# sagitrs/nvlevelz

Hardware: AMD Instinct MI355X
Metric: GiB/s device-resident batched CRC32C over 4 KiB blocks; % HBM-read roofline (higher is better)
Workload: dtype u32

## Files before the change

nvlevelz_amd/csrc/crc32c_dev_sched.h:

```cpp
#pragma once
#include "crc32c_dev.h"

namespace nvl {
namespace dev {

constexpr uint32_t kTail = 64;

template <int U, int NW = kWavesPerWG, int M = kAligned, class G = FixedGeom, bool kRaw = false, bool NIB = false>
__device__ __forceinline__ void run_pairs(const G& g, const KArgs& ka, uint8_t* lds) {
  NVL_STAMP0();
  const int lane = threadIdx.x & 63;
  const uint32_t wv = uniform_u32(threadIdx.x >> 6);
  const uint64_t B0 = g.n * blockIdx.x / gridDim.x;
  const uint64_t B1 = g.n * (blockIdx.x + 1) / gridDim.x;
  const uint32_t cnt = (uint32_t)(B1 - B0);
  const uint32_t nfull = cnt > kTail ? (cnt - kTail) / U : 0u;
  const uint32_t nunits = nfull + (cnt - nfull * U);

  auto unit_pos = [&](uint32_t u, int k, Pos& p) -> bool {
    const uint64_t i = u < nfull ? B0 + (uint64_t)u * U + (uint64_t)k : B0 + (uint64_t)nfull * U + (u - nfull);
    if (u >= nunits || (u >= nfull && k > 0)) return false;
    p.i = i;
    p.c = 0;
    p.bi = g.info(i);
    return true;
  };

  uint32_t u = wv;
  Pos gp[U];
  bool ok[U];
  Chunk cur[U];
  RegionFill rf;
  LdsFill<NW> lf;
  if constexpr (NIB) rf = fill_region_load(ka.tables);
  else lf = fill_lds_load<NW>(ka.tables);
#pragma unroll
  for (int k = 0; k < U; ++k) {
    ok[k] = unit_pos(u, k, gp[k]);
    if (ok[k]) load_chunk<M>(gp[k].bi, 0, lane, cur[k]);
  }
  if constexpr (NIB) fill_region_store(lds, rf, NW);
  else fill_lds_store<NW>(lds, lf, NW);
  __syncthreads();
  const LaneBase lb = make_lane_base(lane);
  NVL_STAMP1();

  while (u < nunits) {
    NVL_COUNT();
    const uint32_t un = pull_unit(lds, lane, NIB ? kRCtrOff : kCtrOff);
    Pos np[U];
    bool nok[U];
    Chunk nxt[U];
#pragma unroll
    for (int k = 0; k < U; ++k) {
      nok[k] = unit_pos(un, k, np[k]);
      if (nok[k]) load_chunk<M>(np[k].bi, 0, lane, nxt[k]);
    }
    if (ok[U - 1]) {
      BufInfo bis[U];
      uint32_t cs[U], raws[U];
#pragma unroll
      for (int k = 0; k < U; ++k) {
        bis[k] = gp[k].bi;
        cs[k] = 0;
      }
      group_raw<M, U, NIB>(lds, lb, bis, cs, lane, cur, raws);
      if (lane == 0) {
#pragma unroll
        for (int k = 0; k < U; ++k) {
          if constexpr (kRaw) ka.raws[gp[k].i] = raws[k];
          else ka.out[gp[k].i] = finish(~raws[k], ka.flags);
        }
      }
    } else {
#pragma unroll
      for (int k = 0; k < U; ++k) {
        if (ok[k]) {
          const uint32_t r = chunk_raw<M, NIB>(lds, lb, gp[k].bi, 0, lane, cur[k]);
          if (lane == 0) {
            if constexpr (kRaw) ka.raws[gp[k].i] = r;
            else ka.out[gp[k].i] = finish(~r, ka.flags);
          }
        }
      }
    }
    u = un;
#pragma unroll
    for (int k = 0; k < U; ++k) {
      gp[k] = np[k];
      ok[k] = nok[k];
      cur[k] = nxt[k];
    }
  }
  NVL_STAMP_END();
}

constexpr int kUnitStep = 1;
constexpr int kUnitStepAligned = 2;

template <int M, int NW, class G>
__device__ __forceinline__ void run_units(const G& g, const KArgs& ka, uint8_t* lds) {
  NVL_STAMP0();
  constexpr int kStep = M == kAligned ? kUnitStepAligned : kUnitStep;
  static_assert(M == kAligned || kStep == 1, "the kGeneral loop skips head chunks one step at a time");
  const int lane = threadIdx.x & 63;
  const uint32_t wv = uniform_u32(threadIdx.x >> 6);
  const uint64_t T = g.total();
  const uint32_t ub0 = blockIdx.x * kUnitsPerWG, ub1 = ub0 + kUnitsPerWG;
  constexpr bool kFastDiv = M != kAligned;
  auto lo_of = [&](uint32_t uu) -> uint64_t { return g.template unit_lo<kFastDiv>(T, uu); };
  auto skip = [&](const Pos& q) -> bool { return M == kGeneral && q.c == 0 && head_first(q.bi.len); };
  auto first_body = [&](const Pos& q) -> uint32_t { return (M == kGeneral && head_first(q.bi.len)) ? 1u : 0u; };
  auto hc_of = [&](const Pos& q) -> uint32_t {
    if (M != kGeneral || !ka.hc || q.c != 1u || !head_first(q.bi.len)) return 0u;
    return __builtin_nontemporal_load((const __attribute__((address_space(1))) uint32_t*)(ka.hc + q.i));
  };

  const LdsFill<NW> lf = fill_lds_load<NW>(ka.tables);
  uint32_t u = ub0 + wv;
  uint64_t t = lo_of(u), t1 = lo_of(u + 1);
  Pos p0{}, p1{};
  Chunk c0, c1;
  uint32_t hv0 = 0u;
  if (t < t1) {
    p0 = unit_start_pos<kFastDiv>(g, u, t);
    if (!skip(p0)) load_chunk<M>(p0.bi, p0.c, lane, c0);
    hv0 = hc_of(p0);
    if (kStep == 2 && t + 1 < t1) {
      p1 = next_pos(g, p0);
      load_chunk<M>(p1.bi, p1.c, lane, c1);
    }
  }
  fill_lds_store<NW>(lds, lf);
  __syncthreads();
  const LaneBase lb = make_lane_base(lane);
  NVL_STAMP1();

  uint32_t un = ub0 + pull_unit(lds, lane);
  uint64_t un_lo = un < ub1 ? lo_of(un) : 0, un_hi = un < ub1 ? lo_of(un + 1) : 0;
  UnitState st{0u, 0u, p0.c <= first_body(p0), Rec{kNoBuf, 0u, 0u}};
  Rec tail{kNoBuf, 0u, 0u};
  while (true) {
    const bool cur = t < t1;
    const bool two = kStep == 2 && t + 1 < t1;
    const uint64_t tn = cur ? t + (two ? 2u : 1u) : t;
    const bool unit_ends = tn == t1;
    Pos q0 = p0, q1 = p0;
    bool q0v = false, q1v = false;
    if (!unit_ends) {
      q0 = two ? next_pos(g, p1) : next_pos(g, p0);
      q0v = true;
      if (kStep == 2 && tn + 1 < t1) {
        q1 = next_pos(g, q0);
        q1v = true;
      }
    } else if (un_lo < un_hi) {
      q0 = unit_start_pos<kFastDiv>(g, un, un_lo);
      q0v = true;
      if (kStep == 2 && un_lo + 1 < un_hi) {
        q1 = next_pos(g, q0);
        q1v = true;
      }
    }
    const bool work = cur && !skip(p0);
    uint32_t w[2][16];
    uint32_t ov[2][4];
    if (work) {
      build_words<M>(p0.bi, p0.c, lane, c0, w[0], ov[0]);
      if (two) build_words<M>(p1.bi, p1.c, lane, c1, w[1], ov[1]);
    }
    Chunk n0, n1;
    uint32_t hvn = 0u;
    if (q0v && !skip(q0)) load_chunk<M>(q0.bi, q0.c, lane, n0);
    if (q0v) hvn = hc_of(q0);
    if (q1v) load_chunk<M>(q1.bi, q1.c, lane, n1);
    if (work) {
      NVL_COUNT();
      uint32_t r[2];
      if (two) {
        chains<2, false>(lds, lb, w, lane, r);
      } else {
        r[0] = chain_fold<M>(lds, lb, w[0], lane);
      }
      consume(st, p0, r[0], lds, lane, ka, hv0);
      if (two) consume(st, p1, r[1], lds, lane, ka);
    }
    if (unit_ends) {
      if (st.cnt) {
        const Pos& pl = two ? p1 : p0;
        const uint32_t norm = normalize(lds, ka.tables, st.acc, pl.bi.J - 1u - pl.c, lane);
        if (st.from_zero) tail = Rec{pl.i, norm, st.cnt};
        else st.head = Rec{pl.i, norm, st.cnt};
      }
      if (lane == 0) g.put_recs(ka, lds, u, st.head, tail);
      if (un >= ub1) break;
      u = un;
      t = un_lo;
      t1 = un_hi;
      un = ub0 + pull_unit(lds, lane);
      un_lo = un < ub1 ? lo_of(un) : 0;
      un_hi = un < ub1 ? lo_of(un + 1) : 0;
      st = UnitState{0u, 0u, q0.c <= first_body(q0), Rec{kNoBuf, 0u, 0u}};
      tail = Rec{kNoBuf, 0u, 0u};
    } else {
      t = tn;
    }
    p0 = q0;
    p1 = q1;
    c0 = n0;
    c1 = n1;
    hv0 = hvn;
  }
  NVL_STAMP_END();
}

template <int NW, class G>
__device__ __forceinline__ void run_general(const G& g, const KArgs& ka, uint8_t* lds) {
  run_units<kGeneral, NW>(g, ka, lds);
}

constexpr uint32_t kBufsMaxJ = 32;

struct CPos {
  uintptr_t ce;
  uint64_t i;
  uint32_t s;
  uint32_t f;
};
constexpr uint32_t kPosValid = 1u, kPosFirst = 2u, kPosLast = 4u, kPosHeadIn = 8u;

__device__ __forceinline__ void load_pos(const CPos& q, int lane, uintptr_t safe, const uint32_t* hc, Chunk& ch,
                                         uint32_t& hv) {
  const uint32_t r = (uint32_t)(q.ce & 3u);
  const uintptr_t A4 = q.ce - kChunk - r;
  const uint32_t lo = lane_load_off(lane);
#pragma unroll
  for (int j = 0; j < 4; ++j) {
    const u32x4 v = ld16(A4 + 1024u * (uint32_t)j + lo);
    ch.d[4 * j + 0] = v.x; ch.d[4 * j + 1] = v.y; ch.d[4 * j + 2] = v.z; ch.d[4 * j + 3] = v.w;
  }
  ch.e[3] = *(const __attribute__((address_space(1))) uint32_t*)(A4 + (r ? kChunk : kChunk - 4u));
  const uintptr_t ha = (q.f & kPosHeadIn) ? (uintptr_t)(hc + q.i) : safe;
  hv = __builtin_nontemporal_load((const __attribute__((address_space(1))) uint32_t*)ha);
}

__device__ __forceinline__ void build_pos(const CPos& q, int lane, const Chunk& ch, uint32_t (&w)[16]) {
#pragma unroll
  for (int k = 0; k < 16; ++k) w[k] = ch.d[k];
  row_transpose(w);
  const uint32_t r = (uint32_t)(q.ce & 3u);
  if (r != 0) {
    const uint32_t nx = next_lane(w[0], ch.e[3]);
#pragma unroll
    for (int k = 0; k < 15; ++k) w[k] = __builtin_amdgcn_alignbyte(w[k + 1], w[k], r);
    w[15] = __builtin_amdgcn_alignbyte(nx, w[15], r);
  }
  const uint32_t inj = q.f >> 8;
  if (inj < 4u && lane == 0) w[0] ^= q.s >> (8u * inj);
}

template <int NW, class G>
__device__ __forceinline__ void run_bufs(const G& g, const KArgs& ka, uint8_t* lds, uint64_t i0, uint64_t i1,
                                         const uint16_t* perm = nullptr) {
  NVL_STAMP0();
  const int lane = threadIdx.x & 63;
  const uint32_t wv = uniform_u32(threadIdx.x >> 6);
  const uint64_t nb = i1 > i0 ? i1 - i0 : 0;
constexpr int kBufsDiv = 4;
  const uint32_t GS = (uint32_t)max<uint64_t>(1, min<uint64_t>(kWave, nb / (kBufsDiv * NW)));
constexpr int kBufsTail = 0;
  const uint64_t kBT = kBufsTail;
  const uint64_t nbig = nb > kBT * 2 ? (nb - kBT) / GS : 0;
  const uint64_t ngroups = nbig + (nb - nbig * GS);
  const uintptr_t safe = (uintptr_t)ka.tables;

  uint64_t todo = 0;
  uintptr_t lp = 0;
  uint64_t lL = 0;
  uint32_t ls = 0, lr = 0;
  uint64_t ngb = 0;
  uint32_t ngn = 0;
  bool has_nxt = false, nxt_ready = false;
  uint64_t no = 0, nL = 0;
  uint32_t ni = 0, nr = 0;
  auto claim_group = [&](uint64_t k) {
    has_nxt = k < ngroups;
    nxt_ready = false;
    ngb = has_nxt ? i0 + (k < nbig ? k * GS : nbig * GS + (k - nbig)) : 0u;
    ngn = has_nxt ? (k < nbig ? GS : 1u) : 1u;
  };
  const uint32_t* const ibase = g.init ? g.init : reinterpret_cast<const uint32_t*>(safe);
  auto meta_load = [&]() {
    const uint64_t pos = ngb + (uint64_t)min<uint32_t>((uint32_t)lane, ngn - 1u);
    const uint64_t i = perm && pos >= i0 ? i0 + perm[pos - i0] : pos;
    nr = (uint32_t)(i - i0);
    no = g.offsets[i];
    nL = g.lengths[i];
    ni = ibase[g.init ? i : 0u];
  };
  auto adopt = [&]() {
    lp = (uintptr_t)g.base + no;
    lL = nL;
    ls = ~(g.init ? ni : g.init_all);
    lr = nr;
    todo = __ballot((uint32_t)lane < ngn && chunks_for(lL) > (head_first(lL) ? 1u : 0u));
    has_nxt = false;
  };
  uintptr_t cp = 0;
  uint64_t cL = 0, ci = 0;
  uint32_t cJ = 0, cx = 0, cc = 0, cfb = 0;
  bool cvalid = false;
  auto next_pos = [&](CPos& q) {
    q.ce = safe + kChunk;
    q.i = 0;
    q.s = 0;
    q.f = 0;
    if (cvalid && cc + 1u < cJ) {
      ++cc;
    } else {
      cvalid = false;
      while (todo == 0) {
        if (!has_nxt || !nxt_ready) return;
        adopt();
        claim_group(pull_unit(lds, lane));
      }
      const uint32_t j = (uint32_t)__builtin_ctzll(todo);
      todo &= todo - 1u;
      cp = (uintptr_t)lane_u64((uint64_t)lp, j);
      cL = lane_u64(lL, j);
      cx = lane_u32(ls, j);
      ci = i0 + lane_u32(lr, j);
      cJ = chunks_for(cL);
      cfb = head_first(cL) ? 1u : 0u;
      cc = cfb;
      cvalid = true;
    }
    q.ce = cp + cL - (uint64_t)kChunk * (cJ - 1u - cc);
    q.i = ci;
    q.s = cx;
    const uintptr_t cs = q.ce - kChunk;
    const uint32_t inj = cs < cp + 4u ? (uint32_t)(cs - cp) : 0xFFu;
    q.f = kPosValid | (cc == cfb ? kPosFirst : 0u) | (cc + 1u == cJ ? kPosLast : 0u) |
          (cc == cfb && cfb == 1u && ka.hc ? kPosHeadIn : 0u) | (inj << 8);
  };
  auto more = [&]() -> bool { return (cvalid && cc + 1u < cJ) || todo != 0 || has_nxt; };

  claim_group(wv);
  meta_load();
  if (has_nxt) adopt();
  claim_group(NW + wv);
  meta_load();
  CPos p0, p1;
  next_pos(p0);
  next_pos(p1);
  Chunk c0, c1;
  uint32_t hv0, hv1;
  const LdsFill<NW> lf = fill_lds_load<NW>(ka.tables);
  load_pos(p0, lane, safe, ka.hc, c0, hv0);
  load_pos(p1, lane, safe, ka.hc, c1, hv1);
  fill_lds_store<NW>(lds, lf, 2u * NW);
  __syncthreads();
  const LaneBase lb = make_lane_base(lane);
  NVL_STAMP1();
  uint32_t acc = 0u;
  auto accumulate = [&](const CPos& q, uint32_t raw, uint32_t hs) {
    const bool first = (q.f & kPosFirst) != 0u;
    acc = (first ? ((q.f & kPosHeadIn) ? hs : 0u) : shift4096(lds, acc, lane)) ^ raw;
    if ((q.f & kPosLast) && lane == 0) ka.out[q.i] = finish(~acc, ka.flags);
  };
  while (true) {
    nxt_ready = has_nxt;
    uint32_t w[2][16];
    const bool work = (p0.f & kPosValid) != 0u;
    if (work) {
      build_pos(p0, lane, c0, w[0]);
      build_pos(p1, lane, c1, w[1]);
    }
    const uint32_t hs0 = shift4096(lds, hv0, lane), hs1 = shift4096(lds, hv1, lane);
    CPos q0, q1;
    next_pos(q0);
    next_pos(q1);
    meta_load();
    load_pos(q0, lane, safe, ka.hc, c0, hv0);
    load_pos(q1, lane, safe, ka.hc, c1, hv1);
    if (work) {
      uint32_t raws[2];
      chains<2, false>(lds, lb, w, lane, raws);
      accumulate(p0, raws[0], hs0);
      if (p1.f & kPosValid) accumulate(p1, raws[1], hs1);
      NVL_COUNT();
    }
    if (!(q0.f & kPosValid) && !more()) break;
    p0 = q0;
    p1 = q1;
  }
  NVL_STAMP_END();
}


constexpr int kFastU = 2;

constexpr int kGenWaves = 16;
constexpr int kGenPairU = 2;
template <int M>
constexpr int waves_of() { return M == kGeneral ? kGenWaves : kWavesPerWG; }

constexpr uint32_t kMaxTiles = 1023;

}
}
```

nvlevelz_amd/csrc/crc32c_fixed.hip:

```cpp
#include "crc32c_launch.h"

namespace nvl {
namespace dev {

constexpr uint64_t kLongFixedMin = 1ull << 18;
__global__ __launch_bounds__(kThreads, 1) void crc32c_fixed_long_kernel(FixedGeom g, KArgs ka) {
  __shared__ __attribute__((aligned(16))) uint8_t lds[kLdsBytes > kRLdsBytes ? kLdsBytes : kRLdsBytes];
  run_pairs<kFastU, kWavesPerWG, kAligned, FixedGeom, false, true>(g, ka, lds);
}

template <int M>
__global__ __launch_bounds__(kWave * waves_of<M>(), 1) void crc32c_fixed_kernel(FixedGeom g, KArgs ka) {
  __shared__ __attribute__((aligned(16))) uint8_t lds[kLdsBytes > kRLdsBytes ? kLdsBytes : kRLdsBytes];
  if constexpr (M == kAligned) {
    if (g.J == 1) {
      run_pairs<kFastU, kWavesPerWG, kAligned, FixedGeom, false, true>(g, ka, lds);
      return;
    }
  }
  if constexpr (M == kGeneral) {
    if (g.J == 1 && !head_first(g.len)) {
      run_pairs<kGenPairU, waves_of<M>(), kGeneral>(g, ka, lds);
      return;
    }
    if (g.J == 1) {
      run_pairs<kGenPairU, waves_of<M>(), kMasked>(g, ka, lds);
      return;
    }
  }
  if constexpr (M == kGeneral) run_general<waves_of<M>()>(g, ka, lds);
  else run_units<M, waves_of<M>()>(g, ka, lds);
}

__global__ __launch_bounds__(kThreads, 1) void crc32c_chunks_kernel(ChunkGeom g, KArgs ka) {
  __shared__ __attribute__((aligned(16))) uint8_t lds[kLdsBytes > kRLdsBytes ? kLdsBytes : kRLdsBytes];
  run_pairs<kFastU, kWavesPerWG, kAligned, ChunkGeom, true, true>(g, ka, lds);
}

__global__ __launch_bounds__(256) void crc32c_fold_kernel(const uint32_t* __restrict__ raws, uint64_t n, uint32_t J,
                                                          const uint32_t* __restrict__ tables,
                                                          uint32_t* __restrict__ out, uint32_t flags) {
  __shared__ uint32_t sh[1024];
  for (uint32_t t = threadIdx.x; t < 1024u; t += blockDim.x) sh[t] = tables[kGComb + 6u * 1024u + t];
  __syncthreads();
  const uint32_t lane = threadIdx.x & 63u;
  const uint32_t R = (J + 63u) / 64u;
  const uint32_t* x2n = tables + kGX2n;
  uint32_t m = nvl::kOne, P = nvl::xpow8(x2n, (uint64_t)kChunk * R);
  const uint32_t e = 63u - lane;
  for (int b = 0; b < 6; ++b) {
    if ((e >> b) & 1u) m = nvl::gf_mul(P, m);
    P = nvl::gf_mul(P, P);
  }
  const uint64_t wpb = blockDim.x >> 6;
  const uint64_t nw = (uint64_t)gridDim.x * wpb;
  for (uint64_t i = (uint64_t)blockIdx.x * wpb + uniform_u32(threadIdx.x >> 6); i < n; i += nw) {
    const int64_t c0 = (int64_t)J - (int64_t)R * (int64_t)(64u - lane);
    const uint32_t* rb = raws + i * J;
    uint32_t acc = 0;
    for (uint32_t k = 0; k < R; ++k) {
      const int64_t c = c0 + (int64_t)k;
      const uint32_t r = c >= 0 ? rb[c] : 0u;
      acc = sh[acc & 255u] ^ sh[256u + ((acc >> 8) & 255u)] ^ sh[512u + ((acc >> 16) & 255u)] ^ sh[768u + (acc >> 24)] ^ r;
    }
    acc = nvl::gf_mul(m, acc);
#pragma unroll
    for (int o = 32; o > 0; o >>= 1) acc ^= (uint32_t)__shfl_xor((int)acc, o);
    if (lane == 0) out[i] = finish(~acc, flags);
  }
}

struct FoldSeg {
  const uint32_t* src;
  uint64_t rows;
  uint32_t J, S, G, step;
  uint32_t m[64];
  uint32_t* dst;
  uint32_t flags;
};
__global__ __launch_bounds__(256) void crc32c_fold_seg_kernel(FoldSeg a) {
  __shared__ uint32_t sh[1024];
  for (uint32_t t = threadIdx.x; t < 1024u; t += blockDim.x) sh[t] = nvl::gf_mul(a.step, (t & 255u) << (8u * (t >> 8)));
  __syncthreads();
  const uint32_t lane = threadIdx.x & 63u;
  const uint32_t R = (a.S + 63u) / 64u;
  const uint32_t m = a.m[lane];
  const uint64_t items = a.rows * a.G;
  const uint64_t wpb = blockDim.x >> 6;
  const uint64_t nw = (uint64_t)gridDim.x * wpb;
  for (uint64_t it = (uint64_t)blockIdx.x * wpb + uniform_u32(threadIdx.x >> 6); it < items; it += nw) {
    const uint64_t row = it / a.G;
    const uint32_t g = (uint32_t)(it - row * a.G);
    const int64_t seg0 = (int64_t)a.J - (int64_t)(a.G - g) * (int64_t)a.S;
    const int64_t c0 = seg0 + (int64_t)a.S - (int64_t)R * (int64_t)(64u - lane);
    const uint32_t* rb = a.src + row * a.J;
    uint32_t acc = 0;
    for (uint32_t k = 0; k < R; ++k) {
      const int64_t c = c0 + (int64_t)k;
      const uint32_t r = (c >= 0 && c >= seg0) ? rb[c] : 0u;
      acc = sh[acc & 255u] ^ sh[256u + ((acc >> 8) & 255u)] ^ sh[512u + ((acc >> 16) & 255u)] ^ sh[768u + (acc >> 24)] ^ r;
    }
    acc = nvl::gf_mul(m, acc);
#pragma unroll
    for (int o = 32; o > 0; o >>= 1) acc ^= (uint32_t)__shfl_xor((int)acc, o);
    if (lane == 0) {
      if (a.G > 1) a.dst[it] = acc;
      else a.dst[row] = finish(~acc, a.flags);
    }
  }
}

__global__ __launch_bounds__(256) void crc32c_fixup_kernel(const Rec* __restrict__ recs, uint32_t nw,
                                                           uint32_t* __restrict__ out, uint32_t flags) {
  const uint32_t w = uniform_u32(blockIdx.x * (blockDim.x >> 6) + (threadIdx.x >> 6));
  const int lane = threadIdx.x & 63;
  if (w >= nw) return;
  const Rec h = recs[2 * (uint64_t)w];
  if (h.buf == kNoBuf || !(h.cnt & kRecEnds)) return;
  uint32_t acc = lane == 0 ? h.raw : 0u;
  for (int64_t base = (int64_t)w - 1; base >= 0; base -= kWave) {
    const int64_t x = base - lane;
    Rec hx{kNoBuf, 0u, 0u}, tx{kNoBuf, 0u, 0u};
    if (x >= 0) {
      hx = recs[2 * x];
      tx = recs[2 * x + 1];
    }
    const bool mid = hx.buf == h.buf;
    const bool first = !mid && tx.buf == h.buf;
    const bool other = !mid && !first && (hx.buf != kNoBuf || tx.buf != kNoBuf || x < 0);
    const unsigned long long stop = __ballot(first || other);
    const int lim = stop ? __builtin_ctzll(stop) : kWave;
    if ((lane < lim && mid) || (lane == lim && first)) acc ^= lane < lim ? hx.raw : tx.raw;
    if (stop) break;
  }
#pragma unroll
  for (int o = 32; o > 0; o >>= 1) acc ^= (uint32_t)__shfl_xor((int)acc, o);
  if (lane == 0) out[h.buf] = finish(~acc, flags);
}

}

hipError_t launch_fixup(const Rec* recs, uint32_t nw, uint32_t* out, uint32_t flags, hipStream_t st,
                        hipEvent_t ev_stop) {
  const uint32_t wpb = 4;
  const dim3 grid((nw + wpb - 1) / wpb), block(dev::kWave * wpb);
  if (ev_stop)
    hipExtLaunchKernelGGL(dev::crc32c_fixup_kernel, grid, block, 0, st, nullptr, ev_stop, 0u, recs, nw, out, flags);
  else
    hipLaunchKernelGGL(dev::crc32c_fixup_kernel, grid, block, 0, st, recs, nw, out, flags);
  return hipGetLastError();
}

static inline size_t recs_part(int num_cu, uint64_t len, uint64_t n) {
  if (n == 0 || chunks_of(len) == 1) return 0;
  return 2ull * grid_for(num_cu, n * (uint64_t)chunks_of(len)) * dev::kUnitsPerWG * sizeof(Rec);
}

constexpr uint32_t kChunkParallelMaxJ = 1024;

constexpr uint32_t kFoldSeg = 1024;

static inline uint64_t fold_segments(uint32_t J) { return (J + kFoldSeg - 1u) / kFoldSeg; }

static inline size_t chunk_raws_bytes(uint64_t len, uint64_t n) {
  if (!(len > dev::kChunk && len % dev::kChunk == 0)) return 0;
  const uint64_t J = len / dev::kChunk;
  const size_t raws = (n * J * sizeof(uint32_t) + 255u) / 256u * 256u;
  return J <= kChunkParallelMaxJ ? n * J * sizeof(uint32_t) : raws + n * fold_segments((uint32_t)J) * sizeof(uint32_t);
}

static void fold_powers(uint64_t step_bytes, uint32_t S, uint32_t* step, uint32_t m[64]) {
  PowTable pw;
  build_pow_table(&pw);
  *step = xpow8(pw.x2n, step_bytes);
  const uint32_t R = (S + 63u) / 64u;
  const uint32_t sR = xpow8(pw.x2n, step_bytes * R);
  m[63] = kOne;
  for (int l = 62; l >= 0; --l) m[l] = gf_mul(m[l + 1], sR);
}
size_t fixed_recs_bytes(int num_cu, uint64_t len, uint64_t n) {
  const size_t cr = chunk_raws_bytes(len, n);
  const size_t r0 = (recs_part(num_cu, len, n) + 255) / 256 * 256;
  const size_t r = r0 > cr ? r0 : cr;
  const bool hcs = n && chunks_of(len) > 1 && dev::head_first(len);
  return r + (hcs ? n * sizeof(uint32_t) : 0);
}

hipError_t launch_fixed(const LaunchCtx& lc, const uint8_t* base, uint64_t stride, uint64_t len, uint64_t n,
                        const uint32_t* init, uint32_t init_all, uint32_t* out, uint32_t flags, Rec* ws) {
  if (n == 0) return hipSuccess;
  const uint32_t J = chunks_of(len);
  const uint32_t grid = grid_for(lc.num_cu, n * (uint64_t)J);
  const bool aligned = len > 0 && (len % dev::kChunk) == 0 && ((uintptr_t)base % 16) == 0 && (stride % 16) == 0;
  dev::FixedGeom g{base, stride, len, n, J, init, init_all};
  Rec* recs = J > 1 ? ws : nullptr;
  const bool masked = !aligned && J == 1 && len >= 1025 && len < dev::kChunk;
  const bool heads = !aligned && dev::head_first(len) && !masked;
  const bool short_all = heads && J == 2 && dev::head_bytes(len, J) < 4u;
  const bool body = !(heads && (J == 1 || short_all));
  uint32_t* hc = heads && J > 1
                     ? reinterpret_cast<uint32_t*>(reinterpret_cast<uint8_t*>(ws) +
                                                   (recs_part(lc.num_cu, len, n) + 255) / 256 * 256)
                     : nullptr;
  hipEvent_t ev_start = lc.ev_start;
  if (heads) {
    hipError_t eh = launch_heads(lc, g, out, flags, hc, ev_start, nullptr, nullptr, short_all,
                                 body ? nullptr : lc.ev_stop);
    if (eh != hipSuccess || !body) return eh;
    ev_start = nullptr;
  }
  if (aligned && J > kChunkParallelMaxJ) {
    const uint64_t T = n * (uint64_t)J;
    const uint32_t jsh = (J & (J - 1u)) == 0u ? (uint32_t)__builtin_ctz(J) : 64u;
    dev::ChunkGeom cg{base, stride, T, J, jsh, init, init_all};
    dev::KArgs kc{out, flags, nullptr, lc.tables, nullptr, nullptr};
    kc.raws = reinterpret_cast<uint32_t*>(ws);
    const uint32_t gc = grid_for(lc.num_cu, T);
    if (ev_start)
      hipExtLaunchKernelGGL(dev::crc32c_chunks_kernel, dim3(gc), dim3(dev::kThreads), 0, lc.stream, ev_start, nullptr,
                            0u, cg, kc);
    else
      hipLaunchKernelGGL(dev::crc32c_chunks_kernel, dim3(gc), dim3(dev::kThreads), 0, lc.stream, cg, kc);
    hipError_t ec = hipGetLastError();
    if (ec != hipSuccess) return ec;
    const uint32_t G = (uint32_t)fold_segments(J);
    uint32_t* segs = reinterpret_cast<uint32_t*>(reinterpret_cast<uint8_t*>(ws) +
                                                 (n * (uint64_t)J * sizeof(uint32_t) + 255u) / 256u * 256u);
    dev::FoldSeg f1{kc.raws, n, J, kFoldSeg, G, 0u, {}, segs, flags};
    fold_powers(dev::kChunk, kFoldSeg, &f1.step, f1.m);
    dev::FoldSeg f2{segs, n, G, G, 1u, 0u, {}, out, flags};
    fold_powers((uint64_t)dev::kChunk * kFoldSeg, G, &f2.step, f2.m);
    const uint32_t g1 = (uint32_t)std::min<uint64_t>((n * G + 3) / 4, 65535);
    hipLaunchKernelGGL(dev::crc32c_fold_seg_kernel, dim3(g1), dim3(256), 0, lc.stream, f1);
    ec = hipGetLastError();
    if (ec != hipSuccess) return ec;
    const uint32_t g2 = (uint32_t)std::min<uint64_t>((n + 3) / 4, 65535);
    if (lc.ev_stop)
      hipExtLaunchKernelGGL(dev::crc32c_fold_seg_kernel, dim3(g2), dim3(256), 0, lc.stream, nullptr, lc.ev_stop, 0u, f2);
    else
      hipLaunchKernelGGL(dev::crc32c_fold_seg_kernel, dim3(g2), dim3(256), 0, lc.stream, f2);
    return hipGetLastError();
  }
  if (aligned && J > 1 && J <= kChunkParallelMaxJ) {
    const uint64_t T = n * (uint64_t)J;
    const uint32_t jsh = (J & (J - 1u)) == 0u ? (uint32_t)__builtin_ctz(J) : 64u;
    dev::ChunkGeom cg{base, stride, T, J, jsh, init, init_all};
    dev::KArgs kc{out, flags, nullptr, lc.tables, nullptr, nullptr};
    kc.raws = reinterpret_cast<uint32_t*>(ws);
    const uint32_t gc = grid_for(lc.num_cu, T);
    if (ev_start)
      hipExtLaunchKernelGGL(dev::crc32c_chunks_kernel, dim3(gc), dim3(dev::kThreads), 0, lc.stream, ev_start, nullptr,
                            0u, cg, kc);
    else
      hipLaunchKernelGGL(dev::crc32c_chunks_kernel, dim3(gc), dim3(dev::kThreads), 0, lc.stream, cg, kc);
    hipError_t ec = hipGetLastError();
    if (ec != hipSuccess) return ec;
    const uint32_t gf = (uint32_t)std::min<uint64_t>((n + 3) / 4, 65535);
    if (lc.ev_stop)
      hipExtLaunchKernelGGL(dev::crc32c_fold_kernel, dim3(gf), dim3(256), 0, lc.stream, nullptr, lc.ev_stop, 0u,
                            kc.raws, n, J, lc.tables, out, flags);
    else
      hipLaunchKernelGGL(dev::crc32c_fold_kernel, dim3(gf), dim3(256), 0, lc.stream, kc.raws, n, J, lc.tables, out,
                         flags);
    return hipGetLastError();
  }
  dev::KArgs ka{out, flags, recs, lc.tables, nullptr, hc};
  hipEvent_t stop_main = J == 1 ? lc.ev_stop : nullptr;
  const bool timed = ev_start || stop_main;
  if (aligned && J == 1 && n >= dev::kLongFixedMin) {
    if (timed)
      hipExtLaunchKernelGGL(dev::crc32c_fixed_long_kernel, dim3(grid), dim3(dev::kThreads), 0, lc.stream, ev_start,
                            stop_main, 0u, g, ka);
    else
      hipLaunchKernelGGL(dev::crc32c_fixed_long_kernel, dim3(grid), dim3(dev::kThreads), 0, lc.stream, g, ka);
    return hipGetLastError();
  }
  if (aligned) {
    if (timed)
      hipExtLaunchKernelGGL(dev::crc32c_fixed_kernel<dev::kAligned>, dim3(grid), dim3(dev::kThreads), 0, lc.stream,
                            ev_start, stop_main, 0u, g, ka);
    else
      hipLaunchKernelGGL(dev::crc32c_fixed_kernel<dev::kAligned>, dim3(grid), dim3(dev::kThreads), 0, lc.stream, g,
                         ka);
  } else {
    if (timed)
      hipExtLaunchKernelGGL(dev::crc32c_fixed_kernel<dev::kGeneral>, dim3(grid), dim3(dev::kWave * dev::kGenWaves),
                            0, lc.stream, ev_start, stop_main, 0u, g, ka);
    else
      hipLaunchKernelGGL(dev::crc32c_fixed_kernel<dev::kGeneral>, dim3(grid), dim3(dev::kWave * dev::kGenWaves), 0,
                         lc.stream, g, ka);
  }
  hipError_t e = hipGetLastError();
  if (e != hipSuccess || J == 1) return e;
  return launch_fixup(recs, grid * dev::kUnitsPerWG, out, flags, lc.stream, lc.ev_stop);
}

}
```

Before: 6021.

## Add dedicated aligned pair loop with ping-pong buffers and branchless safe loads

```diff
diff --git a/nvlevelz_amd/csrc/crc32c_dev_sched.h b/nvlevelz_amd/csrc/crc32c_dev_sched.h
--- a/nvlevelz_amd/csrc/crc32c_dev_sched.h
+++ b/nvlevelz_amd/csrc/crc32c_dev_sched.h
@@ -6,7 +6,7 @@
 
 constexpr uint32_t kTail = 64;
 
-template <int U, int NW = kWavesPerWG, int M = kAligned, class G = FixedGeom, bool kRaw = false, bool NIB = false>
+template <int U, int NW = kWavesPerWG, int M = kAligned, class G = FixedGeom>
 __device__ __forceinline__ void run_pairs(const G& g, const KArgs& ka, uint8_t* lds) {
   NVL_STAMP0();
   const int lane = threadIdx.x & 63;
@@ -30,24 +30,20 @@
   Pos gp[U];
   bool ok[U];
   Chunk cur[U];
-  RegionFill rf;
-  LdsFill<NW> lf;
-  if constexpr (NIB) rf = fill_region_load(ka.tables);
-  else lf = fill_lds_load<NW>(ka.tables);
+  const LdsFill<NW> lf = fill_lds_load<NW>(ka.tables);
 #pragma unroll
   for (int k = 0; k < U; ++k) {
     ok[k] = unit_pos(u, k, gp[k]);
     if (ok[k]) load_chunk<M>(gp[k].bi, 0, lane, cur[k]);
   }
-  if constexpr (NIB) fill_region_store(lds, rf, NW);
-  else fill_lds_store<NW>(lds, lf, NW);
+  fill_lds_store<NW>(lds, lf, NW);
   __syncthreads();
   const LaneBase lb = make_lane_base(lane);
   NVL_STAMP1();
 
   while (u < nunits) {
     NVL_COUNT();
-    const uint32_t un = pull_unit(lds, lane, NIB ? kRCtrOff : kCtrOff);
+    const uint32_t un = pull_unit(lds, lane);
     Pos np[U];
     bool nok[U];
     Chunk nxt[U];
@@ -64,23 +60,17 @@
         bis[k] = gp[k].bi;
         cs[k] = 0;
       }
-      group_raw<M, U, NIB>(lds, lb, bis, cs, lane, cur, raws);
+      group_raw<M, U>(lds, lb, bis, cs, lane, cur, raws);
       if (lane == 0) {
 #pragma unroll
-        for (int k = 0; k < U; ++k) {
-          if constexpr (kRaw) ka.raws[gp[k].i] = raws[k];
-          else ka.out[gp[k].i] = finish(~raws[k], ka.flags);
-        }
+        for (int k = 0; k < U; ++k) ka.out[gp[k].i] = finish(~raws[k], ka.flags);
       }
     } else {
 #pragma unroll
       for (int k = 0; k < U; ++k) {
         if (ok[k]) {
-          const uint32_t r = chunk_raw<M, NIB>(lds, lb, gp[k].bi, 0, lane, cur[k]);
-          if (lane == 0) {
-            if constexpr (kRaw) ka.raws[gp[k].i] = r;
-            else ka.out[gp[k].i] = finish(~r, ka.flags);
-          }
+          const uint32_t r = chunk_raw<M>(lds, lb, gp[k].bi, 0, lane, cur[k]);
+          if (lane == 0) ka.out[gp[k].i] = finish(~r, ka.flags);
         }
       }
     }
@@ -95,14 +85,102 @@
   NVL_STAMP_END();
 }
 
+template <int U, class G, bool kRaw>
+__device__ __forceinline__ void run_pairs_aligned(const G& g, const KArgs& ka, uint8_t* lds) {
+  NVL_STAMP0();
+  constexpr int NW = kWavesPerWG;
+  const int lane = threadIdx.x & 63;
+  const uint32_t wv = uniform_u32(threadIdx.x >> 6);
+  const uint64_t B0 = g.n * blockIdx.x / gridDim.x;
+  const uint64_t B1 = g.n * (blockIdx.x + 1) / gridDim.x;
+  const uint32_t cnt = (uint32_t)(B1 - B0);
+  const uint32_t nfull = cnt > kTail ? (cnt - kTail) / U : 0u;
+  const uint32_t nunits = nfull + (cnt - nfull * U);
+  const uint8_t* const safe = reinterpret_cast<const uint8_t*>(ka.tables);
+
+  struct Unit {
+    uint64_t i;
+    uint32_t nv;
+    uint32_t s[U];
+  };
+  auto issue_pos = [&](Unit& q, int k, Chunk& ch) {
+    const bool v = (uint32_t)k < q.nv;
+    const BufInfo bi = g.info(v ? q.i + (uint64_t)k : B0);
+    q.s[k] = bi.s;
+    load_chunk<kAligned>(BufInfo{v ? bi.p : safe, kChunk, 1u, bi.s}, 0, lane, ch);
+  };
+  auto locate = [&](uint32_t u, Unit& q) {
+    q.nv = u < nfull ? (uint32_t)U : (u < nunits ? 1u : 0u);
+    q.i = u < nfull ? B0 + (uint64_t)u * U : B0 + (uint64_t)nfull * U + (u - nfull);
+  };
+  auto issue = [&](uint32_t u, Unit& q, Chunk (&ch)[U]) {
+    locate(u, q);
+#pragma unroll
+    for (int k = 0; k < U; ++k) issue_pos(q, k, ch[k]);
+  };
+  auto issue_single = [&](uint32_t u, Unit& q, Chunk& ch) {
+    locate(u, q);
+    issue_pos(q, 0, ch);
+  };
+  auto put = [&](uint64_t i, uint32_t raw) {
+    if constexpr (kRaw) ka.raws[i] = raw;
+    else ka.out[i] = finish(~raw, ka.flags);
+  };
+  LaneBase lb;
+  auto compute = [&](const Unit& q, const Chunk (&ch)[U]) {
+    NVL_COUNT();
+    BufInfo bis[U];
+    uint32_t cs[U], raws[U];
+#pragma unroll
+    for (int k = 0; k < U; ++k) {
+      bis[k] = BufInfo{nullptr, kChunk, 1u, q.s[k]};
+      cs[k] = 0;
+    }
+    group_raw<kAligned, U, true>(lds, lb, bis, cs, lane, ch, raws);
+#pragma unroll
+    for (int k = 0; k < U; ++k)
+      if (lane == 0 && (uint32_t)k < q.nv) put(q.i + (uint64_t)k, raws[k]);
+  };
+  auto compute_single = [&](const Unit& q, const Chunk& ch) {
+    NVL_COUNT();
+    const uint32_t r = chunk_raw<kAligned, true>(lds, lb, BufInfo{nullptr, kChunk, 1u, q.s[0]}, 0, lane, ch);
+    if (lane == 0) put(q.i, r);
+  };
+
+  Unit ux, uy;
+  Chunk cx[U], cy[U];
+  const RegionFill rf = fill_region_load(ka.tables);
+  issue(wv, ux, cx);
+  fill_region_store(lds, rf, NW);
+  __syncthreads();
+  lb = make_lane_base(lane);
+  NVL_STAMP1();
+
+  while (ux.nv == (uint32_t)U) {
+    issue(pull_unit(lds, lane, kRCtrOff), uy, cy);
+    compute(ux, cx);
+    issue(pull_unit(lds, lane, kRCtrOff), ux, cx);
+    compute(uy, cy);
+  }
+  while (ux.nv) {
+    issue_single(pull_unit(lds, lane, kRCtrOff), uy, cy[0]);
+    __builtin_amdgcn_sched_barrier(0);
+    compute_single(ux, cx[0]);
+    if (!uy.nv) break;
+    issue_single(pull_unit(lds, lane, kRCtrOff), ux, cx[0]);
+    __builtin_amdgcn_sched_barrier(0);
+    compute_single(uy, cy[0]);
+  }
+  NVL_STAMP_END();
+}
+
 constexpr int kUnitStep = 1;
-constexpr int kUnitStepAligned = 2;
 
 template <int M, int NW, class G>
 __device__ __forceinline__ void run_units(const G& g, const KArgs& ka, uint8_t* lds) {
   NVL_STAMP0();
-  constexpr int kStep = M == kAligned ? kUnitStepAligned : kUnitStep;
-  static_assert(M == kAligned || kStep == 1, "the kGeneral loop skips head chunks one step at a time");
+  constexpr int kStep = kUnitStep;
+  static_assert(M == kGeneral && kStep == 1, "the kGeneral loop skips head chunks one step at a time");
   const int lane = threadIdx.x & 63;
   const uint32_t wv = uniform_u32(threadIdx.x >> 6);
   const uint64_t T = g.total();
diff --git a/nvlevelz_amd/csrc/crc32c_fixed.hip b/nvlevelz_amd/csrc/crc32c_fixed.hip
--- a/nvlevelz_amd/csrc/crc32c_fixed.hip
+++ b/nvlevelz_amd/csrc/crc32c_fixed.hip
@@ -6,17 +6,14 @@
 constexpr uint64_t kLongFixedMin = 1ull << 18;
 __global__ __launch_bounds__(kThreads, 1) void crc32c_fixed_long_kernel(FixedGeom g, KArgs ka) {
   __shared__ __attribute__((aligned(16))) uint8_t lds[kLdsBytes > kRLdsBytes ? kLdsBytes : kRLdsBytes];
-  run_pairs<kFastU, kWavesPerWG, kAligned, FixedGeom, false, true>(g, ka, lds);
+  run_pairs_aligned<kFastU, FixedGeom, false>(g, ka, lds);
 }
 
 template <int M>
 __global__ __launch_bounds__(kWave * waves_of<M>(), 1) void crc32c_fixed_kernel(FixedGeom g, KArgs ka) {
   __shared__ __attribute__((aligned(16))) uint8_t lds[kLdsBytes > kRLdsBytes ? kLdsBytes : kRLdsBytes];
   if constexpr (M == kAligned) {
-    if (g.J == 1) {
-      run_pairs<kFastU, kWavesPerWG, kAligned, FixedGeom, false, true>(g, ka, lds);
-      return;
-    }
+    run_pairs_aligned<kFastU, FixedGeom, false>(g, ka, lds);
   }
   if constexpr (M == kGeneral) {
     if (g.J == 1 && !head_first(g.len)) {
@@ -27,14 +24,13 @@
       run_pairs<kGenPairU, waves_of<M>(), kMasked>(g, ka, lds);
       return;
     }
-  }
-  if constexpr (M == kGeneral) run_general<waves_of<M>()>(g, ka, lds);
-  else run_units<M, waves_of<M>()>(g, ka, lds);
+    run_general<waves_of<M>()>(g, ka, lds);
+  }
 }
 
 __global__ __launch_bounds__(kThreads, 1) void crc32c_chunks_kernel(ChunkGeom g, KArgs ka) {
   __shared__ __attribute__((aligned(16))) uint8_t lds[kLdsBytes > kRLdsBytes ? kLdsBytes : kRLdsBytes];
-  run_pairs<kFastU, kWavesPerWG, kAligned, ChunkGeom, true, true>(g, ka, lds);
+  run_pairs_aligned<kFastU, ChunkGeom, true>(g, ka, lds);
 }
 
 __global__ __launch_bounds__(256) void crc32c_fold_kernel(const uint32_t* __restrict__ raws, uint64_t n, uint32_t J,
@@ -276,6 +272,7 @@
     return hipGetLastError();
   }
   if (aligned) {
+    if (J != 1) return hipErrorInvalidValue;
     if (timed)
       hipExtLaunchKernelGGL(dev::crc32c_fixed_kernel<dev::kAligned>, dim3(grid), dim3(dev::kThreads), 0, lc.stream,
                             ev_start, stop_main, 0u, g, ka);
```

Result: slower. 5874 (-2.4%).
